# nv-tlabs/InfiniCube

Measured on AMD Instinct MI355X. Metric: denoise steps/sec, 93-frame 480p Wan2.1 buffer-conditioned DiT loop, higher is better.
Workload: dtype bf16

## Files before the change

infinicube_amd/csrc/attention.hip:

```cpp
#include "icv_common.h"


int icv_attn1_dispatch(const void* q, int64_t ldq, const void* k, int64_t ldk, const void* v, int64_t ldv, void* o,
                       int64_t ldo, int64_t Sq, int64_t Skv, int64_t heads, float scale, void* stream);
int icv_attn2_dispatch(const void* q, int64_t ldq, const void* k, int64_t ldk, const void* v, int64_t ldv,
                       void* o, int64_t ldo, float* acc, int64_t ldacc, float* ml, int state_in,
                       int state_out, int64_t Sq, int64_t Skv, int64_t heads, float scale, int var,
                       hipStream_t st);

int icv_attn3_dispatch(const void* q, int64_t ldq, const void* k, int64_t ldk, const void* v, int64_t ldv,
                       void* o, int64_t ldo, float* acc, int64_t ldacc, float* ml, int state_in,
                       int state_out, int64_t Sq, int64_t Skv, int64_t heads, float scale, int var,
                       hipStream_t st);

int icv_attn9_dispatch(const void* q, int64_t ldq, const void* k, int64_t ldk, const void* v, int64_t ldv,
                       void* o, int64_t ldo, float* acc, int64_t ldacc, float* ml, int state_in,
                       int state_out, int64_t Sq, int64_t Skv, int64_t heads, float scale, int var,
                       hipStream_t st);
int icv_attn7p_single(const void* q, int64_t ldq, const void* k, int64_t ldk, const void* v, int64_t ldv, void* o, int64_t ldo, float* acc,
                      int64_t ldacc, float* ml, int state_in, int state_out, int64_t Sq, int64_t Skv, int64_t heads, float scale, hipStream_t st);
int icv_attn7q_single(const void* q, int64_t ldq, const void* k, int64_t ldk, const void* v, int64_t ldv, void* o, int64_t ldo, float* acc,
                      int64_t ldacc, float* ml, int state_in, int state_out, int64_t Sq, int64_t Skv, int64_t heads, float scale, int variant,
                      hipStream_t st);
int icv_attn7_dispatch(const void* q, int64_t ldq, const void* k, int64_t ldk, const void* v, int64_t ldv,
                       void* o, int64_t ldo, float* acc, int64_t ldacc, float* ml, int state_in,
                       int state_out, int64_t Sq, int64_t Skv, int64_t heads, float scale, int var,
                       hipStream_t st);
int icv_attn6_dispatch(const void* q, int64_t ldq, const void* k, int64_t ldk, const void* v, int64_t ldv,
                       void* o, int64_t ldo, float* acc, int64_t ldacc, float* ml, int state_in,
                       int state_out, int64_t Sq, int64_t Skv, int64_t heads, float scale, int var,
                       hipStream_t st);
int icv_attn5_dispatch(const void* q, int64_t ldq, const void* k, int64_t ldk, const void* v, int64_t ldv,
                       void* o, int64_t ldo, float* acc, int64_t ldacc, float* ml, int state_in,
                       int state_out, int64_t Sq, int64_t Skv, int64_t heads, float scale, int var,
                       hipStream_t st);
int icv_attn4_dispatch(const void* q, int64_t ldq, const void* k, int64_t ldk, const void* v, int64_t ldv,
                       void* o, int64_t ldo, float* acc, int64_t ldacc, float* ml, int state_in,
                       int state_out, int64_t Sq, int64_t Skv, int64_t heads, float scale, int var,
                       hipStream_t st);

constexpr int ATTN_KERNEL_DEFAULT = 7;
constexpr int ATTN7_VARIANT_DEFAULT = 132;
constexpr int ATTN7Q_DEFAULT = 0;
static int attn_route(const void* q, int64_t ldq, const void* k, int64_t ldk, const void* v, int64_t ldv, void* o,
                      int64_t ldo, float* acc, int64_t ldacc, float* ml, int state_in, int state_out, int64_t Sq,
                      int64_t Skv, int64_t heads, float scale, hipStream_t st) {
#define ATT_ARGS q, ldq, k, ldk, v, ldv, o, ldo, acc, ldacc, ml, state_in, state_out, Sq, Skv, heads, scale
  switch (icv_get_option_int("attn_kernel", ATTN_KERNEL_DEFAULT)) {
    case 7: {
      const int var7 = icv_get_option_int("attn7_variant", -1);
      int short_max = icv_get_option_int("attn7_short", -1);
      if (short_max < 0) short_max = 1024;
      if (var7 < 0 && Skv > short_max && !icv_get_option_int("attn7_plain", 0) && !icv_get_option_int("attn7_ablate", 0) && state_out != 2) {
#ifdef ICV_EXPERIMENTS
        const int q7 = icv_get_option_int("attn7q", ATTN7Q_DEFAULT);
        if (q7 > 0) {
          const int rc = icv_attn7q_single(ATT_ARGS, q7, st);
          if (rc >= 0) return rc;
        }
#endif
        return icv_attn7p_single(ATT_ARGS, st);
      }
      return icv_attn7_dispatch(ATT_ARGS, var7 < 0 ? ATTN7_VARIANT_DEFAULT : var7, st);
    }
#ifdef ICV_EXPERIMENTS
    case 9: return icv_attn9_dispatch(ATT_ARGS, icv_get_option_int("attn9_variant", 0), st);
    case 6: return icv_attn6_dispatch(ATT_ARGS, icv_get_option_int("attn6_variant", 5), st);
    case 5: return icv_attn5_dispatch(ATT_ARGS, 0, st);
    case 4: return icv_attn4_dispatch(ATT_ARGS, icv_get_option_int("attn4_variant", 4), st);
    case 3: return icv_attn3_dispatch(ATT_ARGS, icv_get_option_int("attn3_variant", 0), st);
#else
    case 9: case 6: case 5: case 4: case 3:
      icv_set_error("attn_kernel 3..6 and 9 are experiments: rebuild libicvideo with ICV_EXPERIMENTS=1");
      return 1;
#endif
    default: return icv_attn2_dispatch(ATT_ARGS, icv_get_option_int("attn2_variant", 12), st);
  }
#undef ATT_ARGS
}

extern "C" int icv_attention_fwd_chunk(const void* q, int64_t ldq, const void* k, int64_t ldk,
                                       const void* v, int64_t ldv, void* o, int64_t ldo, float* acc,
                                       int64_t ldacc, float* ml, int64_t Sq, int64_t Skv,
                                       int64_t heads, float scale, int first, int last, void* stream) {
  ICV_REQUIRE(q && k && v, "icv_attention_fwd_chunk: null pointer");
  ICV_REQUIRE(Sq > 0 && Skv > 0 && heads > 0, "icv_attention_fwd_chunk: empty problem");
  ICV_REQUIRE(ldq % 8 == 0 && ldk % 8 == 0 && ldv % 8 == 0, "icv_attention_fwd_chunk: leading dims must keep 16-byte row alignment");
  ICV_REQUIRE((first && last) || (acc && ml && ldacc % 4 == 0), "icv_attention_fwd_chunk: carried state buffers required unless first && last");
  ICV_REQUIRE(!last || (o && ldo % 4 == 0), "icv_attention_fwd_chunk: output required for the last chunk");
  return attn_route(q, ldq, k, ldk, v, ldv, o, ldo, acc, ldacc, ml, first ? 0 : 1, last ? 0 : 1, Sq, Skv, heads, scale, (hipStream_t)stream);
}

extern "C" int icv_attention_fwd(const void* q, int64_t ldq, const void* k, int64_t ldk,
                                 const void* v, int64_t ldv, void* o, int64_t ldo, int64_t Sq,
                                 int64_t Skv, int64_t heads, float scale, void* stream) {
  ICV_REQUIRE(q && k && v && o, "icv_attention_fwd: null pointer");
  ICV_REQUIRE(Sq > 0 && Skv > 0 && heads > 0, "icv_attention_fwd: empty problem (Sq=%lld Skv=%lld heads=%lld)", (long long)Sq, (long long)Skv, (long long)heads);
  ICV_REQUIRE(ldq % 8 == 0 && ldk % 8 == 0 && ldv % 8 == 0 && ldo % 4 == 0, "icv_attention_fwd: leading dims must keep 16-byte row alignment");
  if (icv_get_option_int("attn_kernel", ATTN_KERNEL_DEFAULT) != 1)
    return attn_route(q, ldq, k, ldk, v, ldv, o, ldo, nullptr, 0, nullptr, 0, 0, Sq, Skv, heads, scale, (hipStream_t)stream);
#ifdef ICV_EXPERIMENTS
  return icv_attn1_dispatch(q, ldq, k, ldk, v, ldv, o, ldo, Sq, Skv, heads, scale, stream);
#else
  icv_set_error("attn_kernel 1 is an experiment: rebuild libicvideo with ICV_EXPERIMENTS=1");
  return 1;
#endif
}

extern "C" int icv_attention_fwd_add(const void* q, int64_t ldq, const void* k, int64_t ldk,
                                     const void* v, int64_t ldv, void* o, int64_t ldo, int64_t Sq,
                                     int64_t Skv, int64_t heads, float scale, void* stream) {
  ICV_REQUIRE(q && k && v && o, "icv_attention_fwd_add: null pointer");
  ICV_REQUIRE(Sq > 0 && Skv > 0 && heads > 0, "icv_attention_fwd_add: empty problem (Sq=%lld Skv=%lld heads=%lld)", (long long)Sq, (long long)Skv, (long long)heads);
  ICV_REQUIRE(ldq % 8 == 0 && ldk % 8 == 0 && ldv % 8 == 0 && ldo % 4 == 0, "icv_attention_fwd_add: leading dims must keep 16-byte row alignment");
  return attn_route(q, ldq, k, ldk, v, ldv, o, ldo, nullptr, 0, nullptr, 0, 2, Sq, Skv, heads, scale, (hipStream_t)stream);
}

constexpr int ATTN_MFMA_DEFAULT = 16;
constexpr int ATTN_MFMA_SHORT_DEFAULT = 16;
int icv_attn_mfma(bool short_kv) {
  const int v = icv_get_option_int("attn_mfma", -1);
  if (v < 0) return short_kv ? ATTN_MFMA_SHORT_DEFAULT : ATTN_MFMA_DEFAULT;
  if (v == 16 || v == 32) return v;
  icv_set_error("attn_mfma = %d: the MFMA shape is 16 (16x16x32) or 32 (32x32x16); negative = the default", v);
  return -1;
}

constexpr int ATTN_TILE16_LEAN_DEFAULT = 1;
constexpr int ATTN_TILE16_LEAN_SHORT_DEFAULT = 1;
int icv_attn_tile16_lean(bool short_kv) {
  const int v = icv_get_option_int("attn_tile16_lean", -1);
  if (v < 0) return short_kv ? ATTN_TILE16_LEAN_SHORT_DEFAULT : ATTN_TILE16_LEAN_DEFAULT;
  if (v == 0 || v == 1) return v;
  icv_set_error("attn_tile16_lean = %d: 1 = the lean body of the 16x16x32 tile, 0 = the first body; negative = the default", v);
  return -1;
}

constexpr int ATTN7P_SLIM_DEFAULT = 1;
int icv_attn7p_slim() {
  const int v = icv_get_option_int("attn7p_slim", -1);
  if (v < 0) return ATTN7P_SLIM_DEFAULT;
  if (v == 0 || v == 1) return v;
  icv_set_error("attn7p_slim = %d: 1 = the slim key loop of attn7p, 0 = the one loop; negative = the default", v);
  return -1;
}

namespace {
unsigned long long* g_trace = nullptr;
int g_trace_cap = 0;
}
unsigned long long* icv_attention_trace_buffer(int* capacity) {
  *capacity = g_trace_cap;
  return g_trace;
}
extern "C" int icv_attention_trace(void* buf, int64_t capacity) {
  ICV_REQUIRE(capacity >= 0 && capacity < (1LL << 31), "icv_attention_trace: bad capacity");
  g_trace = (unsigned long long*)buf;
  g_trace_cap = buf ? (int)capacity : 0;
  return 0;
}
```

infinicube_amd/csrc/attn7p.hip:

```cpp
#include <type_traits>
#include "attn_common.h"

namespace att7p {

using attc::D;
using attc::NEG_BIG;
using attc::lds_read_tr16;
constexpr int KVB = 64;
constexpr int TILE_BYTES = KVB * D * 2;
constexpr int STAGE_BYTES = 2 * TILE_BYTES;
constexpr int NST = 4, NW = 8, NI = 16 / NW, QB = NW * 32;
constexpr int LDS_BYTES = NST * STAGE_BYTES + 64;
constexpr int MAX_PIECES = ICV_ATTN_MAX_PIECES;

struct Piece {
  const bf16_t* k;
  const bf16_t* v;
  int rows;
  int flag;
  unsigned value;
  int pad;
};

struct Params {
// ... 290 lines not shown
            if (j >= kb) {
#pragma unroll
              for (int r = 0; r < 16; ++r) st[j][r] -= dm;
            }
#pragma unroll
          for (int r = 0; r < 16; ++r) cinit[r] = -m_new;
        }
        ps = 0.f;
#pragma unroll
        for (int r = 0; r < 16; ++r) {
          const float pv = UNIT ? __builtin_amdgcn_exp2f(st[kb][r]) : __builtin_amdgcn_exp2f(fmaf(st[kb][r], p.sc, mb));
          ps += pv;
          pf[r >> 3][r & 7] = (__bf16)pv;
        }
      }
      psum += ps;
#pragma unroll
      for (int hf = 0; hf < 2; ++hf) {
        const int kk = kb * 2 + hf;
#pragma unroll
        for (int d0 = 0; d0 < 4; ++d0) {
          const int key_l = kk * 16 + v_key_lo;
          const int byte = (d0 * 64 + v_byte_lo) ^ v_sw;
          const bf16x4 va = lds_read_tr16(vs + key_l * 256 + byte);
          const bf16x4 vb = lds_read_tr16(vs + (key_l + 8) * 256 + byte);
          bf16x8 vf;
          vf[0] = va[0]; vf[1] = va[1]; vf[2] = va[2]; vf[3] = va[3];
          vf[4] = vb[0]; vf[5] = vb[1]; vf[6] = vb[2]; vf[7] = vb[3];
          ot[d0] = __builtin_amdgcn_mfma_f32_32x32x16_bf16(vf, pf[hf], ot[d0], 0, 0, 0);
        }
      }
    }
    __builtin_amdgcn_s_setprio(0);
    l_run += psum;
  };

  const int np = FW ? fw_np : __builtin_amdgcn_readfirstlane(pp.n_pieces);
  if constexpr (MF == 16) __builtin_assume(np >= 1);
  unsigned gt = 0;
  unsigned iv = 0;
  P_WAIT_PIECE(0);
  P_SET_DMA_PIECE(0);
  P_DMA_TILE(0, gt);
  P_DMA_TILE(1, gt + 1);
  asm volatile("s_waitcnt vmcnt(0)" ::: "memory");
  P_BARRIER();
  for (int pj = 0; pj < np; ++pj) {
    const int skv = P_ROWS(pj);
    const int nt = (skv + KVB - 1) / KVB;
    if constexpr (MF == 16) __builtin_assume(nt >= 1);
    const unsigned g_next = gt + (unsigned)((nt + 1) & ~1);
    const bool has_next = pj + 1 < np;
    const int nflag = has_next && !FW ? __builtin_amdgcn_readfirstlane(pp.piece[has_next ? pj + 1 : pj].flag) : -1;
    const unsigned nvalue = has_next && !FW ? pp.piece[has_next ? pj + 1 : pj].value : 0u;
    bool next_ready = has_next && nflag < 0;
    bool next_issued = false;
    if (!FW && pp.ptrace && tid == 0) pp.ptrace[(size_t)blockIdx.x * np + pj] = __builtin_amdgcn_s_memrealtime();
    int t_steady = 0;
    if constexpr (SLIM) {
      int t = 0;
      const int t_last = (skv >> 6) - 6;
      if (t_last >= 0) {
        const int64_t kstep = (int64_t)KVB * p.ldk, vstep = (int64_t)KVB * p.ldv;
        const bf16_t* kt_d = kh_d + 2 * kstep;
        const bf16_t* vt_d = vh_d + 2 * vstep;
        const unsigned l_w = lds_base + (unsigned)(wave * NI * 1024);
        unsigned l0_d = l_w + (unsigned)(((gt + 2) & (NST - 1)) * STAGE_BYTES);
        const unsigned l_sum = 2 * l_w + 2 * STAGE_BYTES;
        int yes = 1;
        asm volatile("" : "+s"(yes));
        static_assert(NI == 2, "dma_tile_slim issues two K and two V pieces per wave");
        for (; t <= t_last; t += 2) {
          dma_tile_slim(kt_d, vt_d, ko[0], ko[1], vo[0], vo[1], l0_d);
          dma_tile_slim(kt_d + kstep, vt_d + vstep, ko[0], ko[1], vo[0], vo[1], l0_d + STAGE_BYTES);
          kt_d += 2 * kstep;
          vt_d += 2 * vstep;
          l0_d = l_sum - l0_d;
          tile(std::integral_constant<int, 0>{}, 0, 0, KVB);
          if (yes) tile(std::integral_constant<int, 1>{}, 0, 0, KVB);
          attc::tile16_lean_advance(la16, la16_step);
          la16_step = -la16_step;
          asm volatile("s_waitcnt vmcnt(0)" ::: "memory");
          P_BARRIER();
        }
        t_steady = t;
      }
    }
    for (int t = SLIM ? t_steady : 0; t < nt; t += 2) {
      const bool last_iv = t + 2 >= nt;
      if (!last_iv) {
        P_DMA_TILE(t + 2, gt + t + 2);
        P_DMA_TILE(t + 3, gt + t + 3);
      } else if (has_next && next_ready) {
        P_SET_DMA_PIECE(pj + 1);
        P_DMA_TILE(0, g_next);
        P_DMA_TILE(1, g_next + 1);
        next_issued = true;
      }
      const bool poll = has_next && !next_ready;
      unsigned fv = 0;
      if (poll && wave == 0) fv = load_flag_async(pp.flags + nflag);
      tile(std::integral_constant<int, 0>{}, (int)(gt + t), t * KVB, skv);
      if (t + 1 < nt) tile(std::integral_constant<int, 1>{}, (int)(gt + t + 1), (t + 1) * KVB, skv);
      if constexpr (LEAN) {
        attc::tile16_lean_advance(la16, la16_step);
        la16_step = -la16_step;
      }
      asm volatile("s_waitcnt vmcnt(0)" ::: "memory");
      if (poll && tid == 0) verdict[iv & 1] = (int)(fv - nvalue) >= 0 ? 1u : 0u;
      P_BARRIER();
      if (poll) next_ready = __builtin_amdgcn_readfirstlane(verdict[iv & 1]) != 0;
      ++iv;
    }
    if (!has_next) break;
    if (!next_issued) {
      if (!next_ready) P_WAIT_PIECE(pj + 1);
      P_SET_DMA_PIECE(pj + 1);
      P_DMA_TILE(0, g_next);
      P_DMA_TILE(1, g_next + 1);
      asm volatile("s_waitcnt vmcnt(0)" ::: "memory");
      P_BARRIER();
    }
    gt = g_next;
  }
  asm volatile("s_waitcnt vmcnt(0)" ::: "memory");

  if constexpr (MF == 16) {
    int64_t qr[2];
    int t16 = lane & 15;
    asm volatile("" : "+v"(t16));
#pragma unroll
    for (int qb = 0; qb < 2; ++qb) {
      const int64_t r = q0 + qb * 16 + t16;
      qr[qb] = !FW || r < q_end ? r : p.Sq;
    }
    attc::store_result(p, qr, head, lane >> 4, s16.ot, s16.m_run, s16.l_run);
  } else {
    attc::store_result(p, !FW || q0 + l31 < q_end ? q0 + l31 : p.Sq, head, hi, ot, m_run, l_run);
  }
  if (p.trace && tid == 0 && (int)blockIdx.x < p.trace_cap) {
    unsigned hwid, xcc;
    asm volatile("s_getreg_b32 %0, hwreg(HW_REG_HW_ID)" : "=s"(hwid));
    asm volatile("s_getreg_b32 %0, hwreg(HW_REG_XCC_ID)" : "=s"(xcc));
    unsigned long long* t = p.trace + (size_t)blockIdx.x * 4;
    t[0] = t_start; t[1] = __builtin_amdgcn_s_memrealtime(); t[2] = hwid; t[3] = xcc;
  }
#undef P_ROWS
#undef P_SET_DMA_PIECE
#undef P_DMA_TILE
#undef P_BARRIER
#undef P_WAIT_PIECE
}

template <bool UNIT, bool FW, int MF, bool SLIM = false, bool LEAN = false>
int launch_mf(const Params& pp, hipStream_t st) {
  static icv_dev_flags attr_set = {};
  if (int rc = icv_ensure_dynamic_lds((const void*)attn7p_kernel<UNIT, FW, MF, SLIM, LEAN>, LDS_BYTES, &attr_set, "attn7p")) return rc;
  const int64_t nwg = (int64_t)pp.a.heads * pp.a.nqb;
  hipLaunchKernelGGL((attn7p_kernel<UNIT, FW, MF, SLIM, LEAN>), dim3((unsigned)nwg), dim3(NW * 64), LDS_BYTES, st, pp);
  return icv_check_launch(FW ? "icv_attention_fwd_framewin" : "icv_attention_fwd_pieces");
}

template <bool UNIT, bool FW = false>
int launch(const Params& pp, hipStream_t st) {
  const int mf = icv_attn_mfma(false);
  if (mf < 0) return 1;
  if (mf != 16) return launch_mf<UNIT, FW, 32>(pp, st);
  const int lean = icv_attn_tile16_lean(false);
  if (lean < 0) return 1;
  if (!lean) return launch_mf<UNIT, FW, 16>(pp, st);
  if constexpr (!FW) {
    const int slim = icv_attn7p_slim();
    if (slim < 0) return 1;
    if (slim && pp.a.ldk >= D && pp.a.ldv >= D) return launch_mf<UNIT, FW, 16, true, true>(pp, st);
  }
  return launch_mf<UNIT, FW, 16, false, true>(pp, st);
}

}

extern "C" int icv_attention_fwd_pieces(const void* q, int64_t ldq, const icv_kv_piece* pieces, int64_t n_pieces, int64_t ldk, int64_t ldv,
                                        void* o, int64_t ldo, int64_t Sq, int64_t heads, float scale, const uint32_t* flags, uint32_t* err,
                                        int64_t timeout_us, void* trace, void* stream) {
  ICV_REQUIRE(q && pieces && o, "icv_attention_fwd_pieces: null pointer");
  ICV_REQUIRE(Sq > 0 && heads > 0 && n_pieces > 0, "icv_attention_fwd_pieces: empty problem (Sq=%lld heads=%lld pieces=%lld)", (long long)Sq,
              (long long)heads, (long long)n_pieces);
  ICV_REQUIRE(ldq % 8 == 0 && ldk % 8 == 0 && ldv % 8 == 0 && ldo % 4 == 0, "icv_attention_fwd_pieces: leading dims must keep 16-byte row alignment");
  att7p::Params pp;
  int64_t total = 0;
  int n = 0;
  for (int64_t i = 0; i < n_pieces; ++i) {
    const icv_kv_piece& s = pieces[i];
    ICV_REQUIRE(s.rows >= 0 && s.rows < (1LL << 31) / 64, "icv_attention_fwd_pieces: piece %lld has %lld rows", (long long)i, (long long)s.rows);
    if (s.rows == 0) continue;
    ICV_REQUIRE(n < att7p::MAX_PIECES, "icv_attention_fwd_pieces: more than %d non-empty pieces", att7p::MAX_PIECES);
    ICV_REQUIRE(s.k && s.v, "icv_attention_fwd_pieces: piece %lld has a null pointer", (long long)i);
    ICV_REQUIRE(s.flag < 0 || flags, "icv_attention_fwd_pieces: piece %lld waits for flag %d but no flag array was given", (long long)i, s.flag);
    ICV_REQUIRE(64 * ldk * 2 < (1LL << 32) && 64 * ldv * 2 < (1LL << 32), "icv_attention_fwd_pieces: row stride too large");
    att7p::Piece& d = pp.piece[n++];
    d.k = (const bf16_t*)s.k; d.v = (const bf16_t*)s.v; d.rows = (int)s.rows; d.flag = s.flag; d.value = s.value; d.pad = 0;
    total += s.rows;
  }
  ICV_REQUIRE(n > 0, "icv_attention_fwd_pieces: every piece is empty");
  attc::fill_params(pp.a, q, ldq, nullptr, ldk, nullptr, ldv, o, ldo, nullptr, 0, nullptr, 0, 0, Sq, total, heads, scale, 256);
  pp.a.trace = icv_attention_trace_buffer(&pp.a.trace_cap);
  pp.flags = flags;
  pp.err = err;
  pp.timeout_ticks = timeout_us > 0 ? (unsigned long long)timeout_us * 100ull : 0ull;
  pp.ptrace = (unsigned long long*)trace;
  pp.n_pieces = n;
  hipStream_t st = (hipStream_t)stream;
  return (pp.a.sc == 1.0f && icv_get_option_int("attn_unit_scale", 1)) ? att7p::launch<true>(pp, st) : att7p::launch<false>(pp, st);
}

int icv_attn7p_single(const void* q, int64_t ldq, const void* k, int64_t ldk, const void* v, int64_t ldv, void* o, int64_t ldo, float* acc,
                      int64_t ldacc, float* ml, int state_in, int state_out, int64_t Sq, int64_t Skv, int64_t heads, float scale, hipStream_t st) {
  ICV_REQUIRE(Skv > 0 && Skv < (1LL << 31) / 64 && 64 * ldk * 2 < (1LL << 32) && 64 * ldv * 2 < (1LL << 32), "icv_attention: key axis / row stride too large");
  att7p::Params pp;
  attc::fill_params(pp.a, q, ldq, nullptr, ldk, nullptr, ldv, o, ldo, acc, ldacc, ml, state_in, state_out, Sq, Skv, heads, scale, 256);
  pp.a.trace = icv_attention_trace_buffer(&pp.a.trace_cap);
  pp.flags = nullptr; pp.err = nullptr; pp.timeout_ticks = 0; pp.ptrace = nullptr;
  pp.n_pieces = 1;
  att7p::Piece& d = pp.piece[0];
  d.k = (const bf16_t*)k; d.v = (const bf16_t*)v; d.rows = (int)Skv; d.flag = -1; d.value = 0; d.pad = 0;
  return (pp.a.sc == 1.0f && icv_get_option_int("attn_unit_scale", 1)) ? att7p::launch<true>(pp, st) : att7p::launch<false>(pp, st);
}

extern "C" int icv_attention_fwd_framewin(const void* q, int64_t ldq, const void* k, int64_t ldk, const void* v, int64_t ldv, void* o, int64_t ldo,
                                          int64_t frames, int64_t frame_rows, int64_t heads, int64_t window, int64_t sink, float scale, void* stream) {
  ICV_REQUIRE(q && k && v && o, "icv_attention_fwd_framewin: null pointer");
  ICV_REQUIRE(frames > 0 && frame_rows > 0 && heads > 0, "icv_attention_fwd_framewin: empty problem (frames=%lld frame_rows=%lld heads=%lld)",
              (long long)frames, (long long)frame_rows, (long long)heads);
  ICV_REQUIRE(window >= 0 && sink >= 0, "icv_attention_fwd_framewin: window (%lld) and sink (%lld) must be >= 0", (long long)window, (long long)sink);
  ICV_REQUIRE(sink <= frames, "icv_attention_fwd_framewin: sink (%lld) exceeds the %lld frames", (long long)sink, (long long)frames);
  ICV_REQUIRE(ldq % 8 == 0 && ldk % 8 == 0 && ldv % 8 == 0 && ldo % 4 == 0, "icv_attention_fwd_framewin: leading dims must keep 16-byte row alignment");
  ICV_REQUIRE(frames < (1LL << 31) / 64 && frame_rows < (1LL << 31) / 64 && frames * frame_rows < (1LL << 31) / 64,
              "icv_attention_fwd_framewin: %lld frames of %lld rows: key axis too large", (long long)frames, (long long)frame_rows);
  ICV_REQUIRE(64 * ldk * 2 < (1LL << 32) && 64 * ldv * 2 < (1LL << 32), "icv_attention_fwd_framewin: row stride too large");
  const int64_t nqb = frames * ((frame_rows + att7p::QB - 1) / att7p::QB);
  ICV_REQUIRE(heads * nqb < (1LL << 31), "icv_attention_fwd_framewin: %lld work-groups", (long long)(heads * nqb));
  att7p::Params pp;
  attc::fill_params(pp.a, q, ldq, k, ldk, v, ldv, o, ldo, nullptr, 0, nullptr, 0, 0, frames * frame_rows, frames * frame_rows, heads, scale, 256);
  pp.a.nqb = (int)nqb;
  pp.a.trace = icv_attention_trace_buffer(&pp.a.trace_cap);
  pp.flags = nullptr; pp.err = nullptr; pp.timeout_ticks = 0; pp.ptrace = nullptr;
  pp.n_pieces = 0;
  pp.fw_frames = (int)frames;
  pp.fw_frame_rows = (int)frame_rows;
  pp.fw_window = (int)(window < frames ? window : frames);
  pp.fw_sink = (int)sink;
  hipStream_t st = (hipStream_t)stream;
  return (pp.a.sc == 1.0f && icv_get_option_int("attn_unit_scale", 1)) ? att7p::launch<true, true>(pp, st) : att7p::launch<false, true>(pp, st);
}

namespace {
__global__ void flag_write_kernel(uint32_t* flag, uint32_t value, unsigned long long delay_ticks) {
  if (delay_ticks) {
    const unsigned long long t0 = __builtin_amdgcn_s_memrealtime();
    while (__builtin_amdgcn_s_memrealtime() - t0 < delay_ticks) __builtin_amdgcn_s_sleep(32);
  }
  __hip_atomic_store(flag, value, __ATOMIC_RELEASE, __HIP_MEMORY_SCOPE_SYSTEM);
}
}

extern "C" int icv_flag_write(uint32_t* flags, int64_t index, uint32_t value, int64_t delay_us, void* stream) {
  ICV_REQUIRE(flags && index >= 0, "icv_flag_write: bad argument");
  ICV_REQUIRE(delay_us >= 0 && delay_us <= 10000000, "icv_flag_write: delay_us out of range");
  hipLaunchKernelGGL(flag_write_kernel, dim3(1), dim3(1), 0, (hipStream_t)stream, flags + index, value, (unsigned long long)delay_us * 100ull);
  return icv_check_launch("icv_flag_write");
}
```

infinicube_amd/csrc/attn_common.h:

```cpp
#pragma once
#include "icv_common.h"

unsigned long long* icv_attention_trace_buffer(int* capacity);
int icv_attn_mfma(bool short_kv);
int icv_attn_tile16_lean(bool short_kv);
int icv_attn7p_slim();

namespace attc {

constexpr int D = 128;
constexpr float NEG_BIG = -1.0e30f;

struct Params {
  const bf16_t* q; int64_t ldq;
  const bf16_t* k; int64_t ldk;
  const bf16_t* v; int64_t ldv;
  bf16_t* o; int64_t ldo;
  float* acc; int64_t ldacc;
  float* ml;
  int64_t Sq, Skv;
  int heads, nqb;
  int state_in, state_out;
  float sc;
  float thr;
  int ablate;
  unsigned long long* trace;
  int trace_cap;
};


inline void fill_params(Params& p, const void* q, int64_t ldq, const void* k, int64_t ldk, const void* v,
                        int64_t ldv, void* o, int64_t ldo, float* acc, int64_t ldacc, float* ml, int state_in,
                        int state_out, int64_t Sq, int64_t Skv, int64_t heads, float scale, int rows_per_block) {
  p.q = (const bf16_t*)q; p.ldq = ldq; p.k = (const bf16_t*)k; p.ldk = ldk;
  p.v = (const bf16_t*)v; p.ldv = ldv; p.o = (bf16_t*)o; p.ldo = ldo;
  p.acc = acc; p.ldacc = ldacc; p.ml = ml; p.state_in = state_in; p.state_out = state_out;
  p.Sq = Sq; p.Skv = Skv; p.heads = (int)heads;
  p.nqb = (int)((Sq + rows_per_block - 1) / rows_per_block);
  p.sc = scale * 1.4426950408889634f;
  if (fabsf(p.sc - 1.0f) < 1e-6f) p.sc = 1.0f;
  p.thr = (float)icv_get_option_int("attn_defer_max_log2", 8);
  p.ablate = 0;
  p.trace = nullptr;
  p.trace_cap = 0;
}

typedef __attribute__((address_space(3))) s16x4 lds_s16x4;

__device__ __forceinline__ bf16x4 lds_read_tr16(const char* p) {
  s16x4 r = __builtin_amdgcn_ds_read_tr16_b64_v4i16((lds_s16x4*)(p));
  return __builtin_bit_cast(bf16x4, r);
}

__device__ __forceinline__ void work_item(const Params& p, int& head, int& qb) {
  const int nwg = p.heads * p.nqb;
  const int bid = blockIdx.x;
  const int xcd = bid & 7, local = bid >> 3;
  const int qn = nwg >> 3, r = nwg & 7;
  const int wg = (xcd < r ? xcd * (qn + 1) : r * (qn + 1) + (xcd - r) * qn) + local;
  head = wg / p.nqb;
  qb = wg - head * p.nqb;
}

__device__ __forceinline__ void load_state(const Params& p, int64_t qr_c, int head, int hi, f32x16 (&ot)[4],
                                           float& m_run, float& l_run) {
  if (p.state_in) {
    const float* ap = p.acc + qr_c * p.ldacc + (int64_t)head * D + 4 * hi;
#pragma unroll
    for (int d0 = 0; d0 < 4; ++d0)
#pragma unroll
      for (int rr = 0; rr < 4; ++rr) {
        const float4 a = *reinterpret_cast<const float4*>(ap + d0 * 32 + rr * 8);
        ot[d0][rr * 4 + 0] = a.x; ot[d0][rr * 4 + 1] = a.y; ot[d0][rr * 4 + 2] = a.z; ot[d0][rr * 4 + 3] = a.w;
      }
    const float2 mlv = *reinterpret_cast<const float2*>(p.ml + (qr_c * p.heads + head) * 2);
    m_run = mlv.x;
    l_run = hi == 0 ? mlv.y : 0.f;
  } else {
#pragma unroll
    for (int i = 0; i < 4; ++i)
#pragma unroll
      for (int r = 0; r < 16; ++r) ot[i][r] = 0.f;
    m_run = NEG_BIG;
    l_run = 0.f;
  }
}

__device__ __forceinline__ void store_result(const Params& p, int64_t qr, int head, int hi, const f32x16 (&ot)[4],
                                             float m_run, float l_run) {
  const float l_tot = l_run + __shfl_xor(l_run, 32, 64);
  if (qr >= p.Sq) return;
  if (p.state_out == 1) {
    float* ap = p.acc + qr * p.ldacc + (int64_t)head * D + 4 * hi;
#pragma unroll
    for (int d0 = 0; d0 < 4; ++d0)
#pragma unroll
      for (int rr = 0; rr < 4; ++rr)
        *reinterpret_cast<float4*>(ap + d0 * 32 + rr * 8) =
            make_float4(ot[d0][rr * 4 + 0], ot[d0][rr * 4 + 1], ot[d0][rr * 4 + 2], ot[d0][rr * 4 + 3]);
    if (hi == 0) *reinterpret_cast<float2*>(p.ml + (qr * p.heads + head) * 2) = make_float2(m_run, l_tot);
  } else {
    const float inv = 1.0f / l_tot;
    bf16_t* op = p.o + qr * p.ldo + (int64_t)head * D + 4 * hi;
#pragma unroll
    for (int d0 = 0; d0 < 4; ++d0)
#pragma unroll
      for (int rr = 0; rr < 4; ++rr) {
        float a = ot[d0][rr * 4 + 0] * inv, b = ot[d0][rr * 4 + 1] * inv;
        float c = ot[d0][rr * 4 + 2] * inv, d = ot[d0][rr * 4 + 3] * inv;
        if (p.state_out == 2) {
          const uint2 prev = *reinterpret_cast<const uint2*>(op + d0 * 32 + rr * 8);
          a += __uint_as_float(prev.x << 16); b += __uint_as_float(prev.x & 0xFFFF0000u);
          c += __uint_as_float(prev.y << 16); d += __uint_as_float(prev.y & 0xFFFF0000u);
        }
        *reinterpret_cast<uint2*>(op + d0 * 32 + rr * 8) = make_uint2(pack_bf16x2(a, b), pack_bf16x2(c, d));
      }
  }
}

struct Tile16 {
  f32x4 ot[8][2];
  float m_run[2], l_run[2], m_base[2];
  f32x4 cinit[2];
  bf16x8 qf[2][4];
};

__device__ __forceinline__ void load_state(const Params& p, const int64_t (&qr_c)[2], int head, int g, f32x4 (&ot)[8][2],
                                           float (&m_run)[2], float (&l_run)[2]) {
#pragma unroll
  for (int qb = 0; qb < 2; ++qb) {
    if (p.state_in) {
      const float* ap = p.acc + qr_c[qb] * p.ldacc + (int64_t)head * D + 4 * g;
#pragma unroll
      for (int db = 0; db < 8; ++db) {
        const float4 a = *reinterpret_cast<const float4*>(ap + db * 16);
        ot[db][qb][0] = a.x; ot[db][qb][1] = a.y; ot[db][qb][2] = a.z; ot[db][qb][3] = a.w;
      }
      const float2 mlv = *reinterpret_cast<const float2*>(p.ml + (qr_c[qb] * p.heads + head) * 2);
      m_run[qb] = mlv.x;
      l_run[qb] = g == 0 ? mlv.y : 0.f;
    } else {
#pragma unroll
      for (int db = 0; db < 8; ++db)
#pragma unroll
        for (int r = 0; r < 4; ++r) ot[db][qb][r] = 0.f;
      m_run[qb] = NEG_BIG;
      l_run[qb] = 0.f;
    }
  }
}

__device__ __forceinline__ void store_result(const Params& p, const int64_t (&qr)[2], int head, int g, const f32x4 (&ot)[8][2],
                                             const float (&m_run)[2], const float (&l_run)[2]) {
  float l_tot[2];
#pragma unroll
  for (int qb = 0; qb < 2; ++qb) {
    const float l2 = l_run[qb] + __shfl_xor(l_run[qb], 16, 64);
    l_tot[qb] = l2 + __shfl_xor(l2, 32, 64);
  }
// ... 103 lines not shown
#pragma unroll
      for (int kq = 0; kq < 4; ++kq) T16_KLOAD(kf[kb][kq], kb, kq);
    __builtin_amdgcn_sched_barrier(0);
    if (SETPRIO) __builtin_amdgcn_s_setprio(1);
#pragma unroll
    for (int kq = 0; kq < 4; ++kq)
#pragma unroll
      for (int kb = 0; kb < 4; ++kb) { T16_QK(kb, kq, kf[kb][kq]); }
    if (SETPRIO) __builtin_amdgcn_s_setprio(0);
  } else if (DSMAJOR) {
    constexpr int KD = 3;
    bf16x8 kf[16];
#pragma unroll
    for (int i = 0; i < KD; ++i) T16_KLOAD(kf[i], i & 3, i >> 2);
#pragma unroll
    for (int i = 0; i < 16; ++i) {
      if (i + KD < 16) T16_KLOAD(kf[i + KD], (i + KD) & 3, (i + KD) >> 2);
      T16_QK(i & 3, i >> 2, kf[i]);
    }
    __builtin_amdgcn_sched_group_barrier(0x100, KD, 0);
#pragma unroll
    for (int i = 0; i < 16; ++i) {
      if (i + KD < 16) __builtin_amdgcn_sched_group_barrier(0x100, 1, 0);
      __builtin_amdgcn_sched_group_barrier(0x008, 2, 0);
    }
  } else {
    if (SETPRIO) __builtin_amdgcn_s_setprio(1);
#pragma unroll
    for (int kb = 0; kb < 4; ++kb)
#pragma unroll
      for (int kq = 0; kq < 4; ++kq) {
        bf16x8 kf;
        T16_KLOAD(kf, kb, kq);
        T16_QK(kb, kq, kf);
      }
    if (SETPRIO) __builtin_amdgcn_s_setprio(0);
  }
#undef T16_KADDR
#undef T16_KLOAD
#undef T16_QK
  if (key0 + 64 > skv) {
#pragma unroll
    for (int kb = 0; kb < 4; ++kb)
#pragma unroll
      for (int r = 0; r < 4; ++r) {
        const int64_t key = key0 + kb * 16 + 4 * g + r;
        if (key >= skv) { st[kb][0][r] = NEG_BIG; st[kb][1][r] = NEG_BIG; }
      }
  }
  float one = 1.0f;
  if (LEAN) asm("" : "+s"(one));
  float mb[2] = {-s.m_run[0] * p.sc, -s.m_run[1] * p.sc};
  float psum[2] = {0.f, 0.f};
  if (SETPRIO) __builtin_amdgcn_s_setprio(1);
#pragma unroll
  for (int kk = 0; kk < 2; ++kk) {
    bf16x8 pf[2];
    float ps[2];
#define T16_EXP()                                                                                                   \
  _Pragma("unroll") for (int qb = 0; qb < 2; ++qb) {                                                                \
    ps[qb] = 0.f;                                                                                                   \
    _Pragma("unroll") for (int j = 0; j < 8; ++j) {                                                                 \
      const float sv = st[2 * kk + (j >> 2)][qb][j & 3];                                                            \
      const float pv = UNIT ? __builtin_amdgcn_exp2f(sv) : __builtin_amdgcn_exp2f(fmaf(sv, p.sc, mb[qb]));          \
      if (LEAN && j == 0) ps[qb] = pv;                                                         \
      else if (LEAN && qb == 1) ps[qb] = t16_add_opaque(ps[qb], pv, one);                                           \
      else ps[qb] += pv;                                                                                            \
      pf[qb][j] = (__bf16)pv;                                                                                       \
    }                                                                                                               \
  }
    T16_EXP();
    if (__any(LEAN && UNIT ? !(ps[0] <= la->lim[0]) || !(ps[1] <= la->lim[1]) : !(ps[0] <= p_lim) || !(ps[1] <= p_lim) || no_ref)) {
#pragma unroll
      for (int qb = 0; qb < 2; ++qb) {
        float mloc = st[2 * kk][qb][0];
#pragma unroll
        for (int j = 1; j < 8; ++j) mloc = fmaxf(mloc, st[2 * kk + (j >> 2)][qb][j & 3]);
        mloc = fmaxf(mloc, __shfl_xor(mloc, 16, 64));
        mloc = fmaxf(mloc, __shfl_xor(mloc, 32, 64));
        if (UNIT) mloc += s.m_base[qb];
        const float m_new = fmaxf(s.m_run[qb], mloc);
        const float alpha = __builtin_amdgcn_exp2f((s.m_run[qb] - m_new) * p.sc);
        s.m_run[qb] = m_new;
        if (LEAN && UNIT && kk == 1) la->lim[qb] = m_new < -1.0e29f ? -1.0f : p_lim;
        s.l_run[qb] = (s.l_run[qb] + psum[qb]) * alpha;
        psum[qb] = 0.f;
#pragma unroll
        for (int db = 0; db < 8; ++db)
#pragma unroll
          for (int r = 0; r < 4; ++r) s.ot[db][qb][r] *= alpha;
        mb[qb] = -m_new * p.sc;
        if (UNIT) {
          const float dm = m_new - s.m_base[qb];
          s.m_base[qb] = m_new;
#pragma unroll
          for (int kb = 0; kb < 4; ++kb)
            if (kb >= 2 * kk) {
#pragma unroll
              for (int r = 0; r < 4; ++r) st[kb][qb][r] -= dm;
            }
#pragma unroll
          for (int r = 0; r < 4; ++r) s.cinit[qb][r] = -m_new;
        }
      }
      T16_EXP();
    }
#undef T16_EXP
    if (LEAN) {
      psum[0] = kk == 0 ? ps[0] : psum[0] + ps[0];
      psum[1] = kk == 0 ? ps[1] : t16_add_opaque(psum[1], ps[1], one);
    } else {
      psum[0] += ps[0];
      psum[1] += ps[1];
    }
    constexpr int VD = 2;
    bf16x4 va[8], vb[8];
#define T16_VREAD(DB_)                                                                                  \
  {                                                                                                     \
    if constexpr (LEAN) {                                                                               \
      const unsigned va_a = la->v[DB_] + (unsigned)(STG * 32768 + kk * 8192);                           \
      va[DB_] = __builtin_bit_cast(bf16x4, __builtin_amdgcn_ds_read_tr16_b64_v4i16((lds_s16x4*)(va_a))); \
      vb[DB_] = __builtin_bit_cast(bf16x4, __builtin_amdgcn_ds_read_tr16_b64_v4i16((lds_s16x4*)(va_a + 4096u))); \
    } else {                                                                                            \
      const char* va_p = vs + kk * 8192 + v_row_off + (((DB_) * 32 + v_byte_lo) ^ v_sw);                 \
      va[DB_] = lds_read_tr16(va_p);                                                                    \
      vb[DB_] = lds_read_tr16(va_p + 4096);  \
    }                                                                                                   \
  }
#pragma unroll
    for (int db = 0; db < VD; ++db) T16_VREAD(db);
#pragma unroll
    for (int db = 0; db < 8; ++db) {
      if (db + VD < 8) T16_VREAD(db + VD);
      bf16x8 vf;
      vf[0] = va[db][0]; vf[1] = va[db][1]; vf[2] = va[db][2]; vf[3] = va[db][3];
      vf[4] = vb[db][0]; vf[5] = vb[db][1]; vf[6] = vb[db][2]; vf[7] = vb[db][3];
#pragma unroll
      for (int qb = 0; qb < 2; ++qb) s.ot[db][qb] = __builtin_amdgcn_mfma_f32_16x16x32_bf16(vf, pf[qb], s.ot[db][qb], 0, 0, 0);
    }
#undef T16_VREAD
    __builtin_amdgcn_sched_group_barrier(0x100, 2 * VD, 0);
#pragma unroll
    for (int db = 0; db < 8; ++db) {
      if (db + VD < 8) __builtin_amdgcn_sched_group_barrier(0x100, 2, 0);
      __builtin_amdgcn_sched_group_barrier(0x008, 2, 0);
    }
  }
  if (SETPRIO) __builtin_amdgcn_s_setprio(0);
  s.l_run[0] += psum[0];
  if (LEAN) s.l_run[1] = t16_add_opaque(s.l_run[1], psum[1], one);
  else s.l_run[1] += psum[1];
}

}
```

Baseline: 0.3226.

## Add staggered two-group attn7p kernel overlapping QK^T with softmax across waves

Adds a new attention kernel for single-piece long-key cases. It splits the eight waves into two groups that enter each pipeline slot out of phase: one group starts with QK^T while the other runs softmax plus PV, with barrier placement and DMA issue shifted to match. QK and softmax/PV are split into separate stage-templated helpers, and s_setprio is optionally raised over the softmax/PV section. The goal is to overlap MFMA and VALU/exp work across waves so issue stays busy. In exchange it brings a more complex barrier and DMA schedule, a forced waves_per_eu(2) occupancy hint, and a larger kernel surface.

```diff
diff --git a/infinicube_amd/csrc/attention.hip b/infinicube_amd/csrc/attention.hip
--- a/infinicube_amd/csrc/attention.hip
+++ b/infinicube_amd/csrc/attention.hip
@@ -145,6 +145,32 @@
   return -1;
 }
 
+constexpr int ATTN7P_STAGGER_DEFAULT = 1;
+constexpr int ATTN7P_STAGGER_SETPRIO_DEFAULT = 1;
+constexpr int ATTN7P_STAGGER_SWAP_DEFAULT = 1;
+int icv_attn7p_stagger() {
+  const int v = icv_get_option_int("attn7p_stagger", -1);
+  if (v < 0) return ATTN7P_STAGGER_DEFAULT;
+  if (v == 0 || v == 1) return v;
+  icv_set_error("attn7p_stagger = %d: 1 = the staggered long-key kernel of attn7p, 0 = the slim loop; negative = the default", v);
+  return -1;
+}
+int icv_attn7p_stagger_setprio() {
+  const int v = icv_get_option_int("attn7p_stagger_setprio", -1);
+  if (v < 0) return ATTN7P_STAGGER_SETPRIO_DEFAULT;
+  if (v == 0 || v == 1) return v;
+  icv_set_error("attn7p_stagger_setprio = %d: 1 = s_setprio over softmax + PV in the staggered kernel, 0 = none; negative = the default", v);
+  return -1;
+}
+
+int icv_attn7p_stagger_swap() {
+  const int v = icv_get_option_int("attn7p_stagger_swap", -1);
+  if (v < 0) return ATTN7P_STAGGER_SWAP_DEFAULT;
+  if (v == 0 || v == 1) return v;
+  icv_set_error("attn7p_stagger_swap = %d: 1 = waves 0-3 open a slot with the softmax and waves 4-7 with QK^T, 0 = the other way round; negative = the default", v);
+  return -1;
+}
+
 namespace {
 unsigned long long* g_trace = nullptr;
 int g_trace_cap = 0;
diff --git a/infinicube_amd/csrc/attn7p.hip b/infinicube_amd/csrc/attn7p.hip
--- a/infinicube_amd/csrc/attn7p.hip
+++ b/infinicube_amd/csrc/attn7p.hip
@@ -466,6 +466,175 @@
 #undef P_WAIT_PIECE
 }
 
+template <bool UNIT, bool PRIO, bool SWAP>
+__global__ __launch_bounds__(NW * 64) __attribute__((amdgpu_waves_per_eu(2))) void attn7ps_kernel(Params pp) {
+  const attc::Params& p = pp.a;
+  const float p_lim = __builtin_amdgcn_exp2f(p.thr);
+  extern __shared__ __attribute__((aligned(16))) char smem[];
+  const int tid = threadIdx.x;
+  const int lane = tid & 63;
+  const int wave = __builtin_amdgcn_readfirstlane(tid >> 6);
+
+  int head, qb;
+  attc::work_item(p, head, qb);
+  const int64_t q0 = (int64_t)qb * QB + wave * 32;
+  const unsigned long long t_start = p.trace ? __builtin_amdgcn_s_memrealtime() : 0ull;
+
+  attc::Tile16 s16;
+  int64_t qr16[2];
+#pragma unroll
+  for (int qb = 0; qb < 2; ++qb) {
+    const int64_t r = q0 + qb * 16 + (lane & 15);
+    qr16[qb] = r < p.Sq ? r : p.Sq - 1;
+  }
+  attc::tile16_init<UNIT>(p, qr16, head, lane >> 4, s16);
+  attc::tile16_load_q(p, qr16, head, lane >> 4, s16);
+  __builtin_amdgcn_s_waitcnt(0x0F70);
+
+  static_assert(NI == 2, "dma_tile_slim issues two K and two V pieces per wave");
+  const int pc = lane & 15;
+  const unsigned lds_base = (unsigned)(uintptr_t)((__attribute__((address_space(3))) char*)smem);
+  int dkey[NI], kcol[NI], vcol[NI];
+  unsigned ko[NI], vo[NI];
+#pragma unroll
+  for (int j = 0; j < NI; ++j) {
+    dkey[j] = (wave * NI + j) * 4 + (lane >> 4);
+    kcol[j] = (pc ^ (dkey[j] & 15)) * 8;
+    vcol[j] = attc::tile16_vcol(pc, dkey[j]);
+    ko[j] = (unsigned)(((int64_t)dkey[j] * p.ldk + kcol[j]) * 2) - j * 1024u;
+    vo[j] = (unsigned)(((int64_t)dkey[j] * p.ldv + vcol[j]) * 2) - j * 1024u;
+  }
+  const bf16_t* kh = pp.piece[0].k + (int64_t)head * D;
+  const bf16_t* vh = pp.piece[0].v + (int64_t)head * D;
+  const int skv = __builtin_amdgcn_readfirstlane(pp.piece[0].rows);
+  const int nt = (skv + KVB - 1) / KVB;
+  __builtin_assume(nt >= 1);
+  const int64_t kstep = (int64_t)KVB * p.ldk, vstep = (int64_t)KVB * p.ldv;
+  const unsigned l_w = lds_base + (unsigned)(wave * NI * 1024);
+  auto dma_tile = [&](const int t) __attribute__((always_inline)) {
+    const unsigned l0 = l_w + (unsigned)((t & (NST - 1)) * STAGE_BYTES);
+    if ((t + 1) * KVB <= skv) {
+      dma_tile_slim(kh + (int64_t)t * kstep, vh + (int64_t)t * vstep, ko[0], ko[1], vo[0], vo[1], l0);
+    } else {
+#pragma unroll
+      for (int j = 0; j < NI; ++j) {
+        int64_t r = (int64_t)t * KVB + dkey[j];
+        r = r < skv ? r : skv - 1;
+        dma16(kh + r * p.ldk + kcol[j], l0 + j * 1024);
+        dma16(vh + r * p.ldv + vcol[j], l0 + TILE_BYTES + j * 1024);
+      }
+    }
+  };
+#define S_END_SLOT(N_)                                              \
+  do {                                                              \
+    asm volatile("s_waitcnt vmcnt(" #N_ ") lgkmcnt(0)" ::: "memory"); \
+    __builtin_amdgcn_s_barrier();                                   \
+    asm volatile("" ::: "memory");                                  \
+    __builtin_amdgcn_sched_barrier(0);                              \
+  } while (0)
+#define S_END_SLOT_TAIL(U_)          \
+  do {                               \
+    if ((U_) < nt) S_END_SLOT(4);    \
+    else S_END_SLOT(0);              \
+  } while (0)
+
+  attc::Tile16Addr la16;
+  attc::tile16_lean_addr(lds_base, lane, la16);
+  attc::tile16_lean_lim<UNIT>(s16, p_lim, la16);
+  int la_step = 2 * STAGE_BYTES;
+  f32x4 st[4][2];
+
+  if (pp.ptrace && tid == 0) pp.ptrace[blockIdx.x] = __builtin_amdgcn_s_memrealtime();
+  dma_tile(0);
+  if (nt > 1) dma_tile(1);
+  S_END_SLOT(0);
+  const bool is_b = SWAP ? wave < NW / 2 : wave >= NW / 2;
+  if (is_b && nt > 2) dma_tile(2);
+  const int lead = is_b ? 3 : 2;
+  const bf16_t* kt_d = kh + lead * kstep;
+  const bf16_t* vt_d = vh + lead * vstep;
+  unsigned d0 = l_w + (unsigned)(lead * STAGE_BYTES);
+  unsigned d1 = l_w + (unsigned)(((lead + 1) & (NST - 1)) * STAGE_BYTES);
+  const unsigned d0_sum = 2 * d0 - 2 * STAGE_BYTES, d1_sum = 2 * l_w + (is_b ? 2 : 4) * STAGE_BYTES;
+  const int nfull = skv >> 6;
+  int t = 0;
+  for (; t <= nfull - 5; t += 2) {
+    if (!is_b) dma_tile_slim(kt_d, vt_d, ko[0], ko[1], vo[0], vo[1], d0);
+    attc::tile16_qk<UNIT, 0>(s16, la16, st);
+    if (is_b) {
+      S_END_SLOT(4);
+      dma_tile_slim(kt_d, vt_d, ko[0], ko[1], vo[0], vo[1], d0);
+    }
+    attc::tile16_sv<UNIT, PRIO, 0>(p, p_lim, 0, KVB, lane, s16, la16, st);
+    if (!is_b) {
+      S_END_SLOT(4);
+      dma_tile_slim(kt_d + kstep, vt_d + vstep, ko[0], ko[1], vo[0], vo[1], d1);
+    }
+    attc::tile16_qk<UNIT, 1>(s16, la16, st);
+    if (is_b) {
+      S_END_SLOT(4);
+      dma_tile_slim(kt_d + kstep, vt_d + vstep, ko[0], ko[1], vo[0], vo[1], d1);
+    }
+    attc::tile16_sv<UNIT, PRIO, 1>(p, p_lim, 0, KVB, lane, s16, la16, st);
+    attc::tile16_lean_advance(la16, la_step);
+    la_step = -la_step;
+    kt_d += 2 * kstep;
+    vt_d += 2 * vstep;
+    d0 = d0_sum - d0;
+    d1 = d1_sum - d1;
+    if (!is_b) S_END_SLOT(4);
+  }
+  for (; t < nt; t += 2) {
+    if (!is_b && t + 2 < nt) dma_tile(t + 2);
+    attc::tile16_qk<UNIT, 0>(s16, la16, st);
+    if (is_b) {
+      S_END_SLOT_TAIL(t + 2);
+      if (t + 3 < nt) dma_tile(t + 3);
+    }
+    attc::tile16_sv<UNIT, PRIO, 0>(p, p_lim, (int64_t)t * KVB, skv, lane, s16, la16, st);
+    if (!is_b) S_END_SLOT_TAIL(t + 2);
+    if (t + 1 >= nt) break;
+    if (!is_b && t + 3 < nt) dma_tile(t + 3);
+    attc::tile16_qk<UNIT, 1>(s16, la16, st);
+    if (is_b) {
+      S_END_SLOT_TAIL(t + 3);
+      if (t + 4 < nt) dma_tile(t + 4);
+    }
+    attc::tile16_sv<UNIT, PRIO, 1>(p, p_lim, (int64_t)(t + 1) * KVB, skv, lane, s16, la16, st);
+    attc::tile16_lean_advance(la16, la_step);
+    la_step = -la_step;
+    if (!is_b) S_END_SLOT_TAIL(t + 3);
+  }
+#undef S_END_SLOT
+#undef S_END_SLOT_TAIL
+  asm volatile("s_waitcnt vmcnt(0)" ::: "memory");
+
+  {
+    int64_t qr[2];
+    int t16 = lane & 15;
+    asm volatile("" : "+v"(t16));
+#pragma unroll
+    for (int qb = 0; qb < 2; ++qb) qr[qb] = q0 + qb * 16 + t16;
+    attc::store_result(p, qr, head, lane >> 4, s16.ot, s16.m_run, s16.l_run);
+  }
+  if (p.trace && tid == 0 && (int)blockIdx.x < p.trace_cap) {
+    unsigned hwid, xcc;
+    asm volatile("s_getreg_b32 %0, hwreg(HW_REG_HW_ID)" : "=s"(hwid));
+    asm volatile("s_getreg_b32 %0, hwreg(HW_REG_XCC_ID)" : "=s"(xcc));
+    unsigned long long* tr = p.trace + (size_t)blockIdx.x * 4;
+    tr[0] = t_start; tr[1] = __builtin_amdgcn_s_memrealtime(); tr[2] = hwid; tr[3] = xcc;
+  }
+}
+
+template <bool UNIT, bool PRIO, bool SWAP>
+int launch_stagger(const Params& pp, hipStream_t st) {
+  static icv_dev_flags attr_set = {};
+  if (int rc = icv_ensure_dynamic_lds((const void*)attn7ps_kernel<UNIT, PRIO, SWAP>, NST * STAGE_BYTES, &attr_set, "attn7ps")) return rc;
+  const int64_t nwg = (int64_t)pp.a.heads * pp.a.nqb;
+  hipLaunchKernelGGL((attn7ps_kernel<UNIT, PRIO, SWAP>), dim3((unsigned)nwg), dim3(NW * 64), NST * STAGE_BYTES, st, pp);
+  return icv_check_launch("icv_attention_fwd (staggered)");
+}
+
 template <bool UNIT, bool FW, int MF, bool SLIM = false, bool LEAN = false>
 int launch_mf(const Params& pp, hipStream_t st) {
   static icv_dev_flags attr_set = {};
@@ -486,7 +655,16 @@
   if constexpr (!FW) {
     const int slim = icv_attn7p_slim();
     if (slim < 0) return 1;
-    if (slim && pp.a.ldk >= D && pp.a.ldv >= D) return launch_mf<UNIT, FW, 16, true, true>(pp, st);
+    if (slim && pp.a.ldk >= D && pp.a.ldv >= D) {
+      const int stagger = icv_attn7p_stagger();
+      const int prio = icv_attn7p_stagger_setprio(), swap = icv_attn7p_stagger_swap();
+      if (stagger < 0 || prio < 0 || swap < 0) return 1;
+      if (stagger && pp.n_pieces == 1 && pp.piece[0].flag < 0) {
+        if (swap) return prio ? launch_stagger<UNIT, true, true>(pp, st) : launch_stagger<UNIT, false, true>(pp, st);
+        return prio ? launch_stagger<UNIT, true, false>(pp, st) : launch_stagger<UNIT, false, false>(pp, st);
+      }
+      return launch_mf<UNIT, FW, 16, true, true>(pp, st);
+    }
   }
   return launch_mf<UNIT, FW, 16, false, true>(pp, st);
 }
diff --git a/infinicube_amd/csrc/attn_common.h b/infinicube_amd/csrc/attn_common.h
--- a/infinicube_amd/csrc/attn_common.h
+++ b/infinicube_amd/csrc/attn_common.h
@@ -5,6 +5,9 @@
 int icv_attn_mfma(bool short_kv);
 int icv_attn_tile16_lean(bool short_kv);
 int icv_attn7p_slim();
+int icv_attn7p_stagger();
+int icv_attn7p_stagger_setprio();
+int icv_attn7p_stagger_swap();
 
 namespace attc {
 
@@ -414,4 +417,137 @@
   else s.l_run[1] += psum[1];
 }
 
-}
+template <bool UNIT, int STG>
+__device__ __forceinline__ void tile16_qk(const Tile16& s, const Tile16Addr& la, f32x4 (&st)[4][2]) {
+  static_assert(STG == 0 || STG == 1, "STG: the tile's place in a step of two stages");
+  const f32x4 zero4 = {0.f, 0.f, 0.f, 0.f};
+#define T16_KLOAD(DST_, KB_, KS_) DST_ = *(const lds_bf16x8*)(la.k[KS_] + (unsigned)(STG * 32768 + (KB_) * 4096))
+#define T16_QK(KB_, KS_, KF_)                                                                                       \
+  _Pragma("unroll") for (int qb = 0; qb < 2; ++qb) st[KB_][qb] = __builtin_amdgcn_mfma_f32_16x16x32_bf16(           \
+      KF_, s.qf[qb][KS_], (KS_) == 0 ? (UNIT ? s.cinit[qb] : zero4) : st[KB_][qb], 0, 0, 0)
+  constexpr int KD = 3;
+  bf16x8 kf[16];
+#pragma unroll
+  for (int i = 0; i < KD; ++i) T16_KLOAD(kf[i], i & 3, i >> 2);
+#pragma unroll
+  for (int i = 0; i < 16; ++i) {
+    if (i + KD < 16) T16_KLOAD(kf[i + KD], (i + KD) & 3, (i + KD) >> 2);
+    T16_QK(i & 3, i >> 2, kf[i]);
+  }
+  __builtin_amdgcn_sched_group_barrier(0x100, KD, 0);
+#pragma unroll
+  for (int i = 0; i < 16; ++i) {
+    if (i + KD < 16) __builtin_amdgcn_sched_group_barrier(0x100, 1, 0);
+    __builtin_amdgcn_sched_group_barrier(0x008, 2, 0);
+  }
+#undef T16_KLOAD
+#undef T16_QK
+}
+
+template <bool UNIT, bool SETPRIO, int STG>
+__device__ __forceinline__ void tile16_sv(const Params& p, const float p_lim, const int64_t key0, const int64_t skv, const int lane, Tile16& s,
+                                          Tile16Addr& la, f32x4 (&st)[4][2]) {
+  static_assert(STG == 0 || STG == 1, "STG: the tile's place in a step of two stages");
+  const int g = lane >> 4;
+  if (key0 + 64 > skv) {
+#pragma unroll
+    for (int kb = 0; kb < 4; ++kb)
+#pragma unroll
+      for (int r = 0; r < 4; ++r) {
+        const int64_t key = key0 + kb * 16 + 4 * g + r;
+        if (key >= skv) { st[kb][0][r] = NEG_BIG; st[kb][1][r] = NEG_BIG; }
+      }
+  }
+  float one = 1.0f;
+  asm("" : "+s"(one));
+  float mb[2] = {-s.m_run[0] * p.sc, -s.m_run[1] * p.sc};
+  float psum[2] = {0.f, 0.f};
+  if (SETPRIO) __builtin_amdgcn_s_setprio(1);
+#pragma unroll
+  for (int kk = 0; kk < 2; ++kk) {
+    bf16x8 pf[2];
+    float ps[2];
+#define T16_EXP()                                                                                                   \
+  _Pragma("unroll") for (int qb = 0; qb < 2; ++qb) {                                                                \
+    ps[qb] = 0.f;                                                                                                   \
+    _Pragma("unroll") for (int j = 0; j < 8; ++j) {                                                                 \
+      const float sv = st[2 * kk + (j >> 2)][qb][j & 3];                                                            \
+      const float pv = UNIT ? __builtin_amdgcn_exp2f(sv) : __builtin_amdgcn_exp2f(fmaf(sv, p.sc, mb[qb]));          \
+      if (j == 0) ps[qb] = pv;                                                                 \
+      else if (qb == 1) ps[qb] = t16_add_opaque(ps[qb], pv, one);                                                   \
+      else ps[qb] += pv;                                                                                            \
+      pf[qb][j] = (__bf16)pv;                                                                                       \
+    }                                                                                                               \
+  }
+    T16_EXP();
+    if (__any(UNIT ? !(ps[0] <= la.lim[0]) || !(ps[1] <= la.lim[1]) : !(ps[0] <= p_lim) || !(ps[1] <= p_lim))) {
+#pragma unroll
+      for (int qb = 0; qb < 2; ++qb) {
+        float mloc = st[2 * kk][qb][0];
+#pragma unroll
+        for (int j = 1; j < 8; ++j) mloc = fmaxf(mloc, st[2 * kk + (j >> 2)][qb][j & 3]);
+        mloc = fmaxf(mloc, __shfl_xor(mloc, 16, 64));
+        mloc = fmaxf(mloc, __shfl_xor(mloc, 32, 64));
+        if (UNIT) mloc += s.m_base[qb];
+        const float m_new = fmaxf(s.m_run[qb], mloc);
+        const float alpha = __builtin_amdgcn_exp2f((s.m_run[qb] - m_new) * p.sc);
+        s.m_run[qb] = m_new;
+        if (UNIT && kk == 1) la.lim[qb] = m_new < -1.0e29f ? -1.0f : p_lim;
+        s.l_run[qb] = (s.l_run[qb] + psum[qb]) * alpha;
+        psum[qb] = 0.f;
+#pragma unroll
+        for (int db = 0; db < 8; ++db)
+#pragma unroll
+          for (int r = 0; r < 4; ++r) s.ot[db][qb][r] *= alpha;
+        mb[qb] = -m_new * p.sc;
+        if (UNIT) {
+          const float dm = m_new - s.m_base[qb];
+          s.m_base[qb] = m_new;
+#pragma unroll
+          for (int kb = 0; kb < 4; ++kb)
+            if (kb >= 2 * kk) {
+#pragma unroll
+              for (int r = 0; r < 4; ++r) st[kb][qb][r] -= dm;
+            }
+#pragma unroll
+          for (int r = 0; r < 4; ++r) s.cinit[qb][r] = -m_new;
+        }
+      }
+      T16_EXP();
+    }
+#undef T16_EXP
+    psum[0] = kk == 0 ? ps[0] : psum[0] + ps[0];
+    psum[1] = kk == 0 ? ps[1] : t16_add_opaque(psum[1], ps[1], one);
+    constexpr int VD = 2;
+    bf16x4 va[8], vb[8];
+#define T16_VREAD(DB_)                                                                                  \
+  {                                                                                                     \
+    const unsigned va_a = la.v[DB_] + (unsigned)(STG * 32768 + kk * 8192);                              \
+    va[DB_] = __builtin_bit_cast(bf16x4, __builtin_amdgcn_ds_read_tr16_b64_v4i16((lds_s16x4*)(va_a)));  \
+    vb[DB_] = __builtin_bit_cast(bf16x4, __builtin_amdgcn_ds_read_tr16_b64_v4i16((lds_s16x4*)(va_a + 4096u))); \
+  }
+#pragma unroll
+    for (int db = 0; db < VD; ++db) T16_VREAD(db);
+#pragma unroll
+    for (int db = 0; db < 8; ++db) {
+      if (db + VD < 8) T16_VREAD(db + VD);
+      bf16x8 vf;
+      vf[0] = va[db][0]; vf[1] = va[db][1]; vf[2] = va[db][2]; vf[3] = va[db][3];
+      vf[4] = vb[db][0]; vf[5] = vb[db][1]; vf[6] = vb[db][2]; vf[7] = vb[db][3];
+#pragma unroll
+      for (int qb = 0; qb < 2; ++qb) s.ot[db][qb] = __builtin_amdgcn_mfma_f32_16x16x32_bf16(vf, pf[qb], s.ot[db][qb], 0, 0, 0);
+    }
+#undef T16_VREAD
+    __builtin_amdgcn_sched_group_barrier(0x100, 2 * VD, 0);
+#pragma unroll
+    for (int db = 0; db < 8; ++db) {
+      if (db + VD < 8) __builtin_amdgcn_sched_group_barrier(0x100, 2, 0);
+      __builtin_amdgcn_sched_group_barrier(0x008, 2, 0);
+    }
+  }
+  if (SETPRIO) __builtin_amdgcn_s_setprio(0);
+  s.l_run[0] += psum[0];
+  s.l_run[1] = t16_add_opaque(s.l_run[1], psum[1], one);
+}
+
+}
```

Result: faster. 0.3291 (median of 6 runs) (+2.0%).
